# microsoft/crescent-credentials

Measured on AMD Instinct MI355X. Metric: Groth16 proofs/sec (rs256-sd-shaped circuit, BN254), G1 MSM scalar-adds/sec reported alongside, higher is better.
Workload: dtype u32 limbs (BN254 Fq/Fr, 254-bit modular integers)

## Files before the change

### crescent-credentials_amd/csrc/csr_host.hpp

```cpp
#pragma once
#include <string.h>

#include <algorithm>
#include <unordered_map>
#include <vector>

#include "curve.hpp"
#include "errors.hpp"
#include "host_parallel.hpp"

namespace cg {

static constexpr uint32_t SELL_PIECE = 8;
static constexpr uint32_t SELL_FINAL = 0x80000000u;
static constexpr uint32_t SELL_PAD = 0xffffffffu;

struct HostSellLevel {
    uint32_t n_pieces = 0, n_partials = 0;
    std::vector<uint32_t> slice_ptr;
    RawArray<uint32_t> dst, col, cidx;
    size_t n_slots = 0;
};
struct HostCsr {
    uint64_t rows = 0, nnz = 0;
    std::vector<uint32_t> rp;
    RawArray<uint32_t> idx;
    std::vector<Fr> dict_mont;
    std::vector<uint32_t> long_rows;
    std::vector<HostSellLevel> levels;
    uint32_t sell_scratch = 0;
};

inline std::vector<uint64_t> range_bounds(uint64_t n, uint64_t min_chunk) {
    uint64_t parts = std::min<uint64_t>(host_threads(), (n + min_chunk - 1) / (min_chunk ? min_chunk : 1));
    if (parts < 1) parts = 1;
    std::vector<uint64_t> b(parts + 1);
    for (uint64_t k = 0; k <= parts; ++k) b[k] = n * k / parts;
    return b;
}
template <class Fn>
inline void for_ranges(const std::vector<uint64_t>& bounds, Fn fn) {
    const uint64_t parts = bounds.size() - 1;
    parallel_ranges(parts, 1, [&](uint64_t a, uint64_t b) { for (uint64_t k = a; k < b; ++k) fn(k, bounds[k], bounds[k + 1]); });
}

#ifdef CSR_HOST_TIMING
#include <chrono>
#include <stdio.h>
#define CSR_LAP(name) do { auto _n = std::chrono::steady_clock::now(); fprintf(stderr, "    %-28s %.1f ms\n", name, std::chrono::duration<double, std::milli>(_n - _lap).count()); _lap = _n; } while (0)
#define CSR_LAP_START auto _lap = std::chrono::steady_clock::now()
#else
#define CSR_LAP(name) do {} while (0)
#define CSR_LAP_START do {} while (0)
#endif
namespace csr_detail {
struct Key {
    uint64_t w[4];
    bool operator==(const Key& o) const { return !memcmp(w, o.w, 32); }
};
struct KeyHash {
    size_t operator()(const Key& k) const { return (size_t)(k.w[0] * 0x9e3779b97f4a7c15ull ^ k.w[1] ^ (k.w[2] << 1) ^ (k.w[3] << 7)); }
};
}

inline void csr_build_sell_host(HostCsr& out, const uint32_t* col_h, bool reorder);

inline void csr_prepare_host(const cg_csr& m, uint64_t rows, uint64_t num_variables, bool sliced, bool reorder, HostCsr& out) {
    using namespace csr_detail;
    out.rows = rows;
    out.nnz = m.nnz;
    const uint64_t nnz = m.nnz;
    if (nnz >= (1ull << 32)) throw HipError(CG_ERR_INVALID_ARGUMENT, "matrix with >= 2^32 non-zeros");
    if (m.row_ptr[0] != 0 || m.row_ptr[rows] != nnz) throw HipError(CG_ERR_INVALID_ARGUMENT, "row_ptr does not span [0, nnz]");
    CSR_LAP_START;
    out.rp.resize(rows + 1);
    parallel_ranges(rows + 1, 1u << 16, [&](uint64_t lo, uint64_t hi) {
        for (uint64_t i = lo; i < hi; ++i) {
            if (i && m.row_ptr[i] < m.row_ptr[i - 1]) throw HipError(CG_ERR_INVALID_ARGUMENT, "row_ptr not monotone");
            out.rp[i] = (uint32_t)m.row_ptr[i];
        }
    });
    CSR_LAP("row_ptr");
    out.idx.alloc(nnz);
    uint32_t* idx = out.idx.p;
    const std::vector<uint64_t> tb = range_bounds(nnz, 1u << 16);
// ... 11 lines not shown
            Key key;
            memcpy(key.w, m.coeff + 32 * t, 32);
            if (key.w[0] == 1 && !(key.w[1] | key.w[2] | key.w[3])) { idx[t] = 0; continue; }
            if (have_last && key == last) { idx[t] = last_id; continue; }
            auto it = map.find(key);
            if (it == map.end()) {
                it = map.emplace(key, (uint32_t)keys.size()).first;
                keys.push_back(key);
            }
            last = key; last_id = it->second | 0x80000000u; have_last = true;
            idx[t] = last_id;
        }
    });
    CSR_LAP("local dictionaries");
    std::vector<Fr> dict_h;
    {
        Fr o = Fr::zero(); o.l[0] = 1;
        dict_h.push_back(o);
    }
    constexpr uint32_t MERGE_PARTS = 16;
    std::vector<std::vector<uint32_t>> remap(parts);
    for (uint64_t k = 0; k < parts; ++k) remap[k].resize(local_keys[k].size());
    std::vector<std::vector<Key>> class_keys(MERGE_PARTS);
    std::vector<std::exception_ptr> class_err(MERGE_PARTS);
    parallel_ranges(MERGE_PARTS, 1, [&](uint64_t lo, uint64_t hi) {
        for (uint64_t cls = lo; cls < hi; ++cls) {
            std::unordered_map<Key, uint32_t, KeyHash> mine;
            std::vector<Key>& ck = class_keys[cls];
            for (uint64_t k = 0; k < parts; ++k)
                for (size_t j = 0; j < local_keys[k].size(); ++j) {
                    const Key& key = local_keys[k][j];
                    if ((KeyHash()(key) >> 7) % MERGE_PARTS != cls) continue;
                    auto it = mine.find(key);
                    if (it == mine.end()) {
                        bool lt = false;
                        for (int q = 3; q >= 0; --q) {
                            const uint64_t nq = (uint64_t)FrP::N[2 * q] | ((uint64_t)FrP::N[2 * q + 1] << 32);
                            if (key.w[q] != nq) { lt = key.w[q] < nq; break; }
                        }
                        if (!lt) throw HipError(CG_ERR_INVALID_ARGUMENT, "non-canonical matrix coefficient");
                        it = mine.emplace(key, (uint32_t)ck.size()).first;
                        ck.push_back(key);
                    }
                    remap[k][j] = it->second | ((uint32_t)cls << 27);
                }
        }
    });
    uint32_t class_off[MERGE_PARTS + 1];
    class_off[0] = 1;
    for (uint32_t cls = 0; cls < MERGE_PARTS; ++cls) {
        if (class_keys[cls].size() >= (1u << 27)) throw HipError(CG_ERR_INVALID_ARGUMENT, "too many distinct matrix coefficients");
        class_off[cls + 1] = class_off[cls] + (uint32_t)class_keys[cls].size();
    }
    dict_h.resize(class_off[MERGE_PARTS]);
    parallel_ranges(MERGE_PARTS, 1, [&](uint64_t lo, uint64_t hi) {
        for (uint64_t cls = lo; cls < hi; ++cls)
            for (size_t j = 0; j < class_keys[cls].size(); ++j) memcpy(dict_h[class_off[cls] + j].l, class_keys[cls][j].w, 32);
    });
    for (uint64_t k = 0; k < parts; ++k)
        for (uint32_t& v : remap[k]) v = class_off[v >> 27] + (v & ((1u << 27) - 1));
    CSR_LAP("merge");
    for_ranges(tb, [&](uint64_t k, uint64_t lo, uint64_t hi) {
        const uint32_t* rm = remap[k].data();
        for (uint64_t t = lo; t < hi; ++t)
            if (idx[t] & 0x80000000u) idx[t] = rm[idx[t] & 0x7fffffffu];
    });
    parallel_ranges(dict_h.size(), 1u << 12, [&](uint64_t lo, uint64_t hi) { for (uint64_t i = lo; i < hi; ++i) dict_h[i] = to_mont(dict_h[i]); });
    out.dict_mont.swap(dict_h);
    CSR_LAP("remap + to_mont");
    out.long_rows.clear();
    for (uint64_t i = 0; i < rows; ++i)
        if (out.rp[i + 1] - out.rp[i] > 4096u) out.long_rows.push_back((uint32_t)i);
    out.levels.clear();
    out.sell_scratch = 0;
    CSR_LAP("long rows");
    if (sliced) csr_build_sell_host(out, m.col, reorder);
    CSR_LAP("sliced layout");
}

inline void csr_build_sell_host(HostCsr& out, const uint32_t* col_h, bool reorder) {
    struct Item { uint32_t row, first, len; };
    struct Piece { uint32_t first, len, dst; };
    const uint64_t rows = out.rows, nnz = out.nnz;
    const std::vector<uint32_t>& rp = out.rp;
    CSR_LAP_START;
    RawArray<uint32_t> cur_col, cur_idx;
    cur_col.alloc(nnz);
    cur_idx.alloc(nnz);
    parallel_ranges(nnz, 1u << 18, [&](uint64_t lo, uint64_t hi) {
        memcpy(cur_col.p + lo, col_h + lo, (hi - lo) * 4);
        memcpy(cur_idx.p + lo, out.idx.p + lo, (hi - lo) * 4);
    });
    if (reorder)
        parallel_ranges(rows, 1u << 14, [&](uint64_t lo, uint64_t hi) {
            for (uint64_t i = lo; i < hi; ++i) {
                uint32_t w = rp[i];
                for (uint32_t t = rp[i]; t < rp[i + 1]; ++t)
                    if (cur_idx.p[t] != 0) {
                        std::swap(cur_idx.p[t], cur_idx.p[w]);
                        std::swap(cur_col.p[t], cur_col.p[w]);
                        ++w;
                    }
            }
        });
    CSR_LAP("  copy + reorder");
    RawArray<Item> items;
    size_t n_items = 0;
    {
        const std::vector<uint64_t> rb = range_bounds(rows, 1u << 14);
        std::vector<uint64_t> cnt(rb.size(), 0);
        for_ranges(rb, [&](uint64_t k, uint64_t lo, uint64_t hi) {
            uint64_t c = 0;
            for (uint64_t i = lo; i < hi; ++i) c += rp[i + 1] > rp[i];
            cnt[k + 1] = c;
        });
        for (size_t k = 1; k < cnt.size(); ++k) cnt[k] += cnt[k - 1];
        n_items = cnt.back();
        items.alloc(n_items);
        for_ranges(rb, [&](uint64_t k, uint64_t lo, uint64_t hi) {
            uint64_t at = cnt[k];
            for (uint64_t i = lo; i < hi; ++i)
// ... 30 lines not shown
        next_items.alloc(c_next[nr]);
        RawArray<uint32_t> next_col;
        next_col.alloc(partials);
        for_ranges(ib, [&](uint64_t k, uint64_t lo, uint64_t hi) {
            uint64_t p = c_pieces[k], n = c_next[k], q = c_part[k];
            for (uint64_t i = lo; i < hi; ++i) {
                const Item& it = items.p[i];
                const uint32_t np = (it.len + SELL_PIECE - 1) / SELL_PIECE;
                if (np == 1) {
                    pieces.p[p++] = {it.first, it.len, it.row | SELL_FINAL};
                    continue;
                }
                next_items.p[n++] = {it.row, (uint32_t)q, np};
                for (uint32_t j = 0; j < np; ++j) {
                    const uint32_t b = it.first + j * SELL_PIECE;
                    const uint32_t l = it.len - j * SELL_PIECE < SELL_PIECE ? it.len - j * SELL_PIECE : SELL_PIECE;
                    pieces.p[p++] = {b, l, (uint32_t)q};
                    next_col.p[q] = (uint32_t)q;
                    ++q;
                }
            }
        });
        CSR_LAP("  pieces");
        constexpr uint32_t NK = (SELL_PIECE + 1) * (SELL_PIECE + 1);
        auto key_of = [&](const Piece& p) {
            uint32_t k = 0;
            if (reorder)
                for (uint32_t t = 0; t < p.len; ++t) k += cidx[p.first + t] != 0;
            return (SELL_PIECE - k) * (SELL_PIECE + 1) + (SELL_PIECE - p.len);
        };
        const std::vector<uint64_t> pb = range_bounds(n_pieces, 1u << 13);
        const size_t npr = pb.size() - 1;
        RawArray<uint8_t> keys;
        keys.alloc(n_pieces);
        std::vector<uint64_t> hist((npr + 1) * NK, 0);
        for_ranges(pb, [&](uint64_t k, uint64_t lo, uint64_t hi) {
            uint64_t* h = &hist[k * NK];
            for (uint64_t i = lo; i < hi; ++i) { keys.p[i] = (uint8_t)key_of(pieces.p[i]); h[keys.p[i]]++; }
        });
        {
            uint64_t run = 0;
            for (uint32_t key = 0; key < NK; ++key)
                for (size_t k = 0; k < npr; ++k) { const uint64_t c = hist[k * NK + key]; hist[k * NK + key] = run; run += c; }
        }
        for_ranges(pb, [&](uint64_t k, uint64_t lo, uint64_t hi) {
            uint64_t* h = &hist[k * NK];
            for (uint64_t i = lo; i < hi; ++i) sorted.p[h[keys.p[i]]++] = pieces.p[i];
        });
        CSR_LAP("  sort");
        const uint32_t np = (uint32_t)n_pieces, ns = (np + 63) / 64;
        L.slice_ptr.assign(ns + 1, 0);
        L.dst.alloc(np ? np : 1);
        if (!np) L.dst.p[0] = 0;
        parallel_ranges(ns, 1u << 10, [&](uint64_t lo, uint64_t hi) {
            for (uint64_t s = lo; s < hi; ++s) {
                uint32_t longest = 0;
                for (uint32_t p = (uint32_t)s * 64; p < np && p < ((uint32_t)s + 1) * 64; ++p) longest = std::max(longest, sorted.p[p].len);
                L.slice_ptr[s + 1] = 64 * longest;
            }
        });
        for (uint32_t s = 0; s < ns; ++s) L.slice_ptr[s + 1] += L.slice_ptr[s];
// ... 38 lines not shown
```

### crescent-credentials_amd/csrc/field29.hpp

```cpp
#pragma once
#include "field.hpp"

namespace cg {

static constexpr uint32_t M29 = (1u << 29) - 1u;

struct Fq29P {
    static constexpr uint32_t N[9] = {0x187cfd47u, 0x010460b6u, 0x1c72a34fu, 0x02d522d0u, 0x1585d978u,
                                      0x02db40c0u, 0x00a6e141u, 0x0e5c2634u, 0x0030644eu};
    static constexpr uint32_t NINV = 0x04866389u;
    static constexpr uint32_t ONE[9] = {0x157ccc21u, 0x141c2758u, 0x185230d3u, 0x014c0419u, 0x0aa36fb9u,
                                        0x1d4240ceu, 0x11d54c07u, 0x052ac7a8u, 0x000dc836u};
    static constexpr uint32_t R2[9] = {0x059bac10u, 0x0d1503a3u, 0x018016b8u, 0x10ab0ca8u, 0x02632639u,
                                       0x02c0169fu, 0x169bfd53u, 0x11869d4cu, 0x002a11a6u};
    static constexpr uint32_t C256[9] = {0x13349ca1u, 0x1a5d84a8u, 0x0a3e5cacu, 0x100249e0u, 0x12b951e8u,
                                         0x0e92d304u, 0x14cb95b3u, 0x041b9d3du, 0x00058003u};
    typedef FqP P256;
};
struct Fr29P {
    static constexpr uint32_t N[9] = {0x10000001u, 0x1f0fac9fu, 0x0e5c2450u, 0x07d090f3u, 0x1585d283u,
                                      0x02db40c0u, 0x00a6e141u, 0x0e5c2634u, 0x0030644eu};
    static constexpr uint32_t NINV = 0x0fffffffu;
    static constexpr uint32_t ONE[9] = {0x0fffff57u, 0x1ea70ab4u, 0x052c068bu, 0x17504f49u, 0x0aa8075bu,
                                        0x1d4240ceu, 0x11d54c07u, 0x052ac7a8u, 0x000dc836u};
// ... 233 lines not shown
    pack29(t, r.l);
    return r;
}

using Fq29 = F29<Fq29P>;
using Fr29 = F29<Fr29P>;

CG_HD Fr29 weak_reduce(const Fr29& v) {
    constexpr uint32_t MU = 88753990u;
    const uint32_t q = (uint32_t)(((uint64_t)v.l[8] * MU) >> 48);
    const int32_t nq = -(int32_t)q;
    Fr29 r;
    int64_t c = 0;
#pragma unroll
    for (int i = 0; i < 9; ++i) {
        c += (int64_t)v.l[i];
        c += (int64_t)nq * (int64_t)(int32_t)Fr29P::N[i];
        if (i < 8) { r.l[i] = (uint32_t)c & M29; c >>= 29; }
        else r.l[i] = (uint32_t)c;
    }
    return r;
}

CG_HD void bfly(Fr29& u, Fr29& v, const Fr29& w) {
    Fr29 t = mul(v, w);
    v = sub<3, 1>(u, t);
    u = add(u, t);
}

template <class P>
struct S29 {
    int32_t l[9];
    CG_HD static S29 from_unsigned(const F29<P>& a) {
        S29 r;
#pragma unroll
        for (int i = 0; i < 9; ++i) r.l[i] = (int32_t)a.l[i];
        return r;
    }
    CG_HD static S29 one() { return from_unsigned(F29<P>::one()); }
};
struct NoFuse { CG_HD void operator()(int, int64_t&) const {} };
template <class P>
struct FuseMul1 {
    const S29<P>& x; int32_t s;
    CG_HD void operator()(int j, int64_t& c) const { c += (int64_t)x.l[j] * (int64_t)s; }
};
// ... 235 lines not shown
```

### crescent-credentials_amd/csrc/ntt.hip

```cpp

#include "ntt.hpp"

#include <algorithm>

namespace cg {

Fr fr_from_u64(uint64_t v) {
    Fr a = Fr::zero();
    a.l[0] = (uint32_t)v;
    a.l[1] = (uint32_t)(v >> 32);
    return to_mont(a);
}
Fr fr_pow_u64(const Fr& a, uint64_t e) {
    Fr r = Fr::one();
    for (int b = 63; b >= 0; --b) {
        r = sqr(r);
        if ((e >> b) & 1ull) r = mul(r, a);
    }
    return r;
}
Fr fr_root_of_unity(int logn) {
    uint32_t e[8];
    uint32_t nm1[8];
    for (int i = 0; i < 8; ++i) nm1[i] = FrP::N[i];
// ... 83 lines not shown
            uint64_t pos = cur[m.col[t]]++;
            out.row[pos] = (uint32_t)i;
            memcpy(&out.coeff[pos * 32], m.coeff + 32 * t, 32);
        }
    out.view.row_ptr = out.ptr.data();
    out.view.col = out.row.data();
    out.view.coeff = out.coeff.data();
    out.view.nnz = m.nnz;
}


void DevCsr::upload(const cg_csr& m, uint64_t rows_, uint64_t num_variables, hipStream_t st, bool sliced) {
    static const bool plain = CG_TUNE_ENV("SELL_PLAIN") != nullptr;
    HostCsr h;
    csr_prepare_host(m, rows_, num_variables, sliced, !plain, h);
    rows = rows_;
    nnz = m.nnz;
    row_ptr.alloc(rows + 1);
    n_long_rows = h.long_rows.size();
    long_rows.alloc(h.long_rows.size() ? h.long_rows.size() : 1);
    col.alloc(nnz ? nnz : 1);
    coef_idx.alloc(nnz ? nnz : 1);
    dict.alloc(h.dict_mont.size());
    auto h2d = [&](void* dst, const void* src, size_t bytes) { if (bytes) CG_HIP(hipMemcpyAsync(dst, src, bytes, hipMemcpyHostToDevice, st)); };
    h2d(long_rows.p, h.long_rows.data(), h.long_rows.size() * 4);
    h2d(row_ptr.p, h.rp.data(), (rows + 1) * 4);
    h2d(col.p, m.col, nnz * 4);
    h2d(coef_idx.p, h.idx.p, nnz * 4);
    h2d(dict.p, h.dict_mont.data(), h.dict_mont.size() * sizeof(Fr));
    n_sell = (int)h.levels.size();
    sell_scratch = h.sell_scratch;
    for (int k = 0; k < n_sell; ++k) {
        const HostSellLevel& H = h.levels[k];
        SellLevel& L = sell[k];
        L.n_pieces = H.n_pieces;
        L.n_partials = H.n_partials;
        L.slice_ptr.alloc(H.slice_ptr.size()); L.col.alloc(H.n_slots); L.cidx.alloc(H.n_slots); L.dst.alloc(H.dst.size());
        h2d(L.slice_ptr.p, H.slice_ptr.data(), H.slice_ptr.size() * 4);
        h2d(L.col.p, H.col.p, H.n_slots * 4);
        h2d(L.cidx.p, H.cidx.p, H.n_slots * 4);
        h2d(L.dst.p, H.dst.p, H.dst.size() * 4);
    }
    CG_HIP(hipStreamSynchronize(st));
}

static constexpr uint32_t SPMV_LONG_ROW = 4096;

__global__ void __launch_bounds__(256) k_spmv(const uint32_t* __restrict__ row_ptr, const uint32_t* __restrict__ col,
                                              const uint32_t* __restrict__ cidx, const Fr* __restrict__ dict,
                                              const Fr* __restrict__ w, Fr* __restrict__ out, uint64_t rows) {
    uint64_t i = (uint64_t)blockIdx.x * blockDim.x + threadIdx.x;
    if (i >= rows) return;
// ... 45 lines not shown
```

### crescent-credentials_amd/csrc/ntt.hpp

```cpp
#pragma once
#include "common.hpp"
#include "csr_host.hpp"

namespace cg {

struct NttDomain {
    int logn = 0;
    uint64_t n = 0;
    DevBuf<Fr> tw_fwd;
    DevBuf<Fr> tw_inv;
    DevBuf<Fr> coset_br;
    DevBuf<Fr> icoset_br;
    Fr vanishing_inv;
    void build(int logn, bool with_coset, hipStream_t st);
};

Fr fr_from_u64(uint64_t v);
Fr fr_pow_u64(const Fr& a, uint64_t e);
Fr fr_root_of_unity(int logn);

void fr_pow_table(Fr* out, const Fr& base, const Fr& scale, uint64_t n, bool bitrev, int logn, hipStream_t st);

struct SellLevel {
    uint32_t n_pieces = 0, n_partials = 0;
    DevBuf<uint32_t> slice_ptr;
    DevBuf<uint32_t> col;
    DevBuf<uint32_t> cidx;
    DevBuf<uint32_t> dst;
};

struct DevCsr {
    uint64_t rows = 0, nnz = 0;
    DevBuf<uint32_t> row_ptr;
    DevBuf<uint32_t> long_rows;
    uint64_t n_long_rows = 0;
    DevBuf<uint32_t> col;
    DevBuf<uint32_t> coef_idx;
    DevBuf<Fr> dict;
    SellLevel sell[8];
    int n_sell = 0;
    uint32_t sell_scratch = 0;
    void upload(const cg_csr& m, uint64_t rows, uint64_t num_variables, hipStream_t st, bool sliced = true);
};
struct HostCsc {
    std::vector<uint64_t> ptr;
    std::vector<uint32_t> row;
    std::vector<uint8_t> coeff;
    cg_csr view;
};
void csr_transpose(const cg_csr& m, uint64_t rows, uint64_t cols, HostCsc& out);

void spmv(const DevCsr& m, const Fr* w, Fr* out, hipStream_t st);

}
```

### crescent-credentials_amd/csrc/prover.hip

```cpp
#include <atomic>
#include <condition_variable>
#include <shared_mutex>
#include <memory>
#include <mutex>
#include <chrono>
#include <cstdlib>
#include <exception>
#include <functional>
#include <thread>

#include "msm.hpp"
#include "ntt.hpp"
#include "scalar_form.hpp"
#include "wmap29.hpp"

namespace cg {

const char* csr_view_problem(const cg_csr& m);

std::string& last_error() {
    static thread_local std::string e;
    return e;
}
int fail(int code, const char* fmt, ...) {
// ... 721 lines not shown
                    c->b_same_identities = v1 == v2;
                }
            }
        }
        for (const MatJob& j : mj)
            if (j.err) std::rethrow_exception(j.err);
        for (int k = 0; k < 3; ++k) {
            c->matrix_bytes += mj[k].bytes;
            c->lt.matrices_ms = std::max(c->lt.matrices_ms, mj[k].ms);
        }
        {
            AllocScope booking(&c->matrix_bytes);
            if (!c->external_q) {
                c->wdom.build(c->dom, s0);
                if (c->h_strided) c->wstr.build(c->dom, ilog2_ceil((uint64_t)c->shard_count), c->shard_rank, s0);
                c->dA.build(c->A, s0); c->dB.build(c->B, s0); c->dC.build(c->C, s0);
            }
            CG_HIP(hipStreamSynchronize(s0));
            if (c->external_q) {
                c->A = DevCsr(); c->B = DevCsr(); c->C = DevCsr();
            }
            c->dom.tw_fwd.release(); c->dom.tw_inv.release(); c->dom.coset_br.release(); c->dom.icoset_br.release();
            c->A.dict.release(); c->B.dict.release(); c->C.dict.release();
        }
        c->latency = n_slots == 1;
        if (opt && (opt->flags & CG_FLAG_LATENCY_MODE)) c->latency = true;
        if (opt && (opt->flags & CG_FLAG_THROUGHPUT_MODE)) c->latency = false;
        c->spin_wait = opt && (opt->flags & CG_FLAG_SPIN_WAIT);
        if (const char* e = CG_TUNE_ENV("LATENCY_MODE")) c->latency = e[0] == '1';
        const auto t_slots = std::chrono::steady_clock::now();
        const int n_now = staged ? std::min(n_slots, 4) : n_slots;
        if (staged) c->folded = false;
        SlotRecipe slot_recipe;
        for (int k = 0; k < n_now; ++k) c->slots.push_back(make_slot(c.get(), c->tables, s0, slot_recipe));
        CG_HIP(hipStreamSynchronize(s0));
        const char* hwq_env = getenv("GPU_MAX_HW_QUEUES");
        const int hwq = (opt && opt->hw_queues > 0) ? opt->hw_queues : (hwq_env ? atoi(hwq_env) : 4);
        const size_t n_copy_streams = hwq >= n_slots + 4 ? 4 : (size_t)n_slots + 2;
        for (int k = 0; k < n_slots + 2; ++k) {
            if (c->up_streams.size() < n_copy_streams) {
                hipStream_t us = nullptr;
                CG_HIP(hipStreamCreateWithFlags(&us, hipStreamNonBlocking));
                c->up_streams.push_back(us);
            }
            std::unique_ptr<Upload> u(new Upload());
            u->w.alloc(M);
// ... 809 lines not shown
```

### crescent-credentials_amd/csrc/unit.hip

```cpp
#include <chrono>
#include <memory>
#include <mutex>
#include <thread>

#include "host_parallel.hpp"
#include "msm.hpp"
#include "scalar_form.hpp"
#include "wmap29.hpp"

using namespace cg;

struct cg_msm_ctx {
    int device = 0;
    int group = 1;
    uint64_t n = 0;
    bool mont_scalars = false;
    MsmBases<Fq> b1;
    MsmBases<Fq2> b2;
    MsmEngine<Fq> e1;
    MsmEngine<Fq2> e2;
    DevBuf<Fr> scalars;
    DevBuf<uint32_t> bad;
    PinnedBuf<uint32_t> h_bad;
    hipStream_t st = nullptr;
// ... 237 lines not shown
    if (logD > 28)
        return fail(CG_ERR_POLY_DEGREE_TOO_LARGE, "num_constraints + num_inputs = %llu exceeds 2^28",
                    (unsigned long long)(num_constraints + num_inputs));
    try {
        int dev = device;
        if (dev < 0) CG_HIP(hipGetDevice(&dev));
        CG_HIP(hipSetDevice(dev));
        std::unique_ptr<cg_qap_ctx> c(new cg_qap_ctx());
        c->device = dev;
        c->l = num_inputs; c->m = num_constraints; c->M = num_variables;
        c->logD = logD; c->D = 1ull << logD;
        CG_HIP(hipStreamCreateWithFlags(&c->st, hipStreamNonBlocking));
        for (auto& e : c->ev) CG_HIP(hipEventCreate(&e));
        c->A.upload(abc[0], c->m, c->M, c->st);
        c->B.upload(abc[1], c->m, c->M, c->st);
        c->C.upload(abc[2], c->m, c->M, c->st);
        c->dom.build(logD, true, c->st);
        CG_HIP(hipStreamSynchronize(c->st));
        c->wdom.build(c->dom, c->st);
        c->dA.build(c->A, c->st); c->dB.build(c->B, c->st); c->dC.build(c->C, c->st);
        CG_HIP(hipStreamSynchronize(c->st));
        c->dom.tw_fwd.release(); c->dom.tw_inv.release(); c->dom.coset_br.release(); c->dom.icoset_br.release();
        c->A.dict.release(); c->B.dict.release(); c->C.dict.release();
        c->wm.alloc(c->M, c->D, std::max(c->A.sell_scratch, std::max(c->B.sell_scratch, c->C.sell_scratch)));
        c->w_canon.alloc(c->M);
        c->h_canon.alloc(c->D);
        c->mont_scalars = scalar_form == CG_FORM_MONTGOMERY;
        if (c->mont_scalars) c->form_bad.alloc(1);
        *out = c.release();
        return CG_OK;
    } catch (...) {
        return translate_current_exception();
    }
}

extern "C" uint64_t cg_qap_domain_size(const cg_qap_ctx* ctx) { return ctx ? ctx->D : 0; }

static const char* const BAD_ASSIGNMENT = "full_assignment holds a value >= the scalar field modulus";

static const Fr* qap_assignment(cg_qap_ctx* ctx, const void* full_assignment, int on_device) {
    const Fr* w = (const Fr*)full_assignment;
    if (!on_device) {
        CG_HIP(hipMemcpyAsync(ctx->w_canon.p, full_assignment, ctx->M * 32, hipMemcpyHostToDevice, ctx->st));
        w = ctx->w_canon.p;
    }
    if (ctx->mont_scalars) {
// ... 247 lines not shown
```

### crescent-credentials_amd/csrc/wmap29.hip

```cpp
#include "wmap29.hpp"
#include "satcheck.hpp"

namespace cg {

static constexpr int TS29_SMALL = 10, TS29_BIG = 11;
static int strided_max_stages(int tile_log) { return tile_log == TS29_BIG ? 10 : 6; }
static int ntt_passes(int logn, int tile_log) {
    if (logn <= tile_log) return 1;
    const int smax = strided_max_stages(tile_log);
    return 1 + (logn - tile_log + smax - 1) / smax;
}
static int ntt_tile_log(int logn) {
    static const int forced = [] {
        const char* e = CG_TUNE_ENV("NTT_TILE");
        return (e && (atoi(e) == TS29_SMALL || atoi(e) == TS29_BIG)) ? atoi(e) : 0;
    }();
    if (forced) return (forced == TS29_BIG && logn > TS29_SMALL) ? TS29_BIG : TS29_SMALL;
    return (logn >= 20 && ntt_passes(logn, TS29_BIG) < ntt_passes(logn, TS29_SMALL)) ? TS29_BIG : TS29_SMALL;
}

__device__ __forceinline__ Fr29 load_packed29(const uint32_t* __restrict__ base, uint64_t idx) {
    const uint4* p = reinterpret_cast<const uint4*>(base + idx * 8);
    uint4 a = p[0], b = p[1];
    uint32_t w[8] = {a.x, a.y, a.z, a.w, b.x, b.y, b.z, b.w};
// ... 73 lines not shown
    const Fr s = mul(fr_from_u64(5), fr_pow_u64(fr_root_of_unity(big.logn), (uint64_t)rank));
    DevBuf<Fr> t(big.n);
    fr_pow_table(t.p, s, inv(fr_from_u64(big.n)), big.n, false, big.logn, st);
    fold.alloc(big.n * 8);
    k_to_packed29<<<ceil_div(big.n, 256), 256, 0, st>>>(t.p, fold.p, big.n, 0, 0);
    CG_KERNEL_CHECK();
    CG_HIP(hipStreamSynchronize(st));
}

__global__ void __launch_bounds__(256) k_fold29(const uint32_t* __restrict__ a, const uint32_t* __restrict__ T, uint32_t* __restrict__ out,
                                                uint32_t d, int logd, uint32_t terms) {
    const uint32_t i = blockIdx.x * blockDim.x + threadIdx.x;
    if (i >= d) return;
    Fr29 acc = Fr29::zero();
    for (uint32_t t = 0; t < terms; ++t) {
        const uint64_t e = (uint64_t)i + (uint64_t)t * d;
        acc = add(acc, mul(load_packed29(a, e), load_packed29(T, e)));
        if ((t & 3u) == 3u) acc = normalize(acc);
        if ((t & 63u) == 63u) acc = weak_reduce(acc);
    }
    store_packed29(out, brev(i, logd), weak_reduce(normalize(acc)));
}

void Csr29::build(const DevCsr& m, hipStream_t st) {
    dict.alloc(m.dict.n * 8);
    k_to_packed29<<<ceil_div(m.dict.n, 256), 256, 0, st>>>(m.dict.p, dict.p, m.dict.n, 0, 0);
    CG_KERNEL_CHECK();
}

__device__ __forceinline__ bool fr_lt_modulus(const Fr& x) {
    bool lt = false, decided = false;
#pragma unroll
    for (int k = 7; k >= 0; --k) {
        if (!decided && x.l[k] != FrP::N[k]) { lt = x.l[k] < FrP::N[k]; decided = true; }
    }
    return lt;
}

__global__ void __launch_bounds__(256) k_w_to29(const Fr* __restrict__ w, uint32_t* __restrict__ out, uint64_t n,
                                                uint32_t* __restrict__ bad_input, uint32_t* __restrict__ va, uint64_t m, uint64_t l, int logn) {
    uint64_t i = (uint64_t)blockIdx.x * blockDim.x + threadIdx.x;
    if (i >= n) return;
    Fr x = w[i];
    if (!fr_lt_modulus(x)) *bad_input = 1u;
    const Fr29 v = mul(unpack29<Fr29P>(x.l), Fr29::from_limbs(Fr29P::R2));
    store_packed29(out, i, v);
    if (i < l) store_packed29(va, brev((uint32_t)(m + i), logn), v);
}


__global__ void __launch_bounds__(256) k_sell29(const uint32_t* __restrict__ slice_ptr, const uint32_t* __restrict__ col,
                                                const uint32_t* __restrict__ cidx, const uint32_t* __restrict__ dst,
                                                const uint32_t* __restrict__ dict, const uint32_t* __restrict__ src,
                                                uint32_t* __restrict__ out, uint32_t* __restrict__ scratch, uint32_t n_pieces, int logn) {
    const uint32_t p = blockIdx.x * blockDim.x + threadIdx.x;
    if (p >= n_pieces) return;
    const uint32_t s = p >> 6, lane = p & 63u;
    const uint32_t base = slice_ptr[s], len = (slice_ptr[s + 1] - base) >> 6;
    Fr29 acc = Fr29::zero();
    uint32_t cnt = 0;
#if !defined(CG_SELL_BATCH)
#define CG_SELL_BATCH 0
#endif
#if CG_SELL_BATCH == 0
    for (uint32_t t = 0; t < len; ++t) {
        const uint32_t ci = cidx[base + t * 64 + lane];
        if (ci == SELL_PAD) continue;
        Fr29 v = load_packed29(src, col[base + t * 64 + lane]);
        if (ci != 0) v = mul(v, load_packed29(dict, ci));
        acc = add(acc, v);
        if ((++cnt & 3u) == 0) acc = normalize(acc);
    }
#else
    constexpr uint32_t BS = CG_SELL_BATCH;
    uint32_t ci[SELL_PIECE], cl[SELL_PIECE];
#pragma unroll
    for (uint32_t t = 0; t < SELL_PIECE; ++t) {
        const bool in = t < len;
        ci[t] = in ? cidx[base + t * 64 + lane] : SELL_PAD;
        cl[t] = in ? col[base + t * 64 + lane] : 0u;
    }
#pragma unroll
    for (uint32_t h = 0; h < SELL_PIECE; h += BS) {
        if (h >= len) break;
        uint4 rv[BS][2], rd[BS][2];
#pragma unroll
        for (uint32_t u = 0; u < BS; ++u) {
            const uint32_t t = h + u;
            if (ci[t] == SELL_PAD) continue;
            const uint4* pv = reinterpret_cast<const uint4*>(src + (uint64_t)cl[t] * 8);
            rv[u][0] = pv[0]; rv[u][1] = pv[1];
            if (ci[t] != 0) {
                const uint4* pd = reinterpret_cast<const uint4*>(dict + (uint64_t)ci[t] * 8);
                rd[u][0] = pd[0]; rd[u][1] = pd[1];
            }
        }
#pragma unroll
        for (uint32_t u = 0; u < BS; ++u) {
            const uint32_t t = h + u;
            if (ci[t] == SELL_PAD) continue;
            const uint32_t wv[8] = {rv[u][0].x, rv[u][0].y, rv[u][0].z, rv[u][0].w, rv[u][1].x, rv[u][1].y, rv[u][1].z, rv[u][1].w};
            Fr29 v = unpack29<Fr29P>(wv);
            if (ci[t] != 0) {
                const uint32_t wd[8] = {rd[u][0].x, rd[u][0].y, rd[u][0].z, rd[u][0].w, rd[u][1].x, rd[u][1].y, rd[u][1].z, rd[u][1].w};
                v = mul(v, unpack29<Fr29P>(wd));
            }
            acc = add(acc, v);
            if ((++cnt & 3u) == 0) acc = normalize(acc);
        }
    }
#endif
    const uint32_t d = dst[p];
    const Fr29 r = weak_reduce(normalize(acc));
    if (d & SELL_FINAL) store_packed29(out, brev(d & ~SELL_FINAL, logn), r);
    else store_packed29(scratch, d, r);
}

struct Pass29 {
    int logn, ts, S, cbits, gbit_lo, q0;
};
__device__ __forceinline__ uint32_t l2g29(uint32_t e, uint32_t tile, const Pass29& pp) {
    const int extra_bits = pp.ts - pp.S - pp.cbits;
    uint32_t colv = e & ((1u << pp.cbits) - 1u);
    uint32_t g = (e >> pp.cbits) & ((1u << pp.S) - 1u);
    uint32_t extra = e >> (pp.cbits + pp.S);
    uint32_t T = (tile << extra_bits) | extra;
    const int lo_bits = pp.gbit_lo - pp.cbits;
    uint32_t Tlo = T & ((1u << lo_bits) - 1u);
    uint32_t Thi = T >> lo_bits;
    return colv | (Tlo << pp.cbits) | (g << pp.gbit_lo) | (Thi << (pp.gbit_lo + pp.S));
}
__device__ __forceinline__ uint32_t lds_off(uint32_t e) { return e * 9u + (e >> 5); }
__device__ __forceinline__ Fr29 lds_get(const uint32_t* s, uint32_t e) {
    Fr29 r;
    const uint32_t o = lds_off(e);
#pragma unroll
// ... 217 lines not shown
}

static void wm29_products(const Wm29Domain& dom, const DevCsr& A, const DevCsr& B, const DevCsr& C, const Csr29& dA, const Csr29& dB,
                          const Csr29& dC, Wm29Buffers& buf, const Fr* w_canon, uint64_t M, uint64_t m, uint64_t l, hipStream_t st, int nvec,
                          int half) {
    const uint64_t D = dom.n;
    const int logn = dom.logn;
    buf.h_bad_input.p[0] = 0;
    uint32_t* v[3] = {buf.va.p, buf.vb.p, buf.vc.p};
    fill_zero(v[0], D * 32, st);
    k_w_to29<<<ceil_div(M, 256), 256, 0, st>>>(w_canon, buf.w29.p, M, buf.h_bad_input.dev(), buf.va.p, m, l, logn);
    CG_KERNEL_CHECK();
    const DevCsr* mats[3] = {&A, &B, &C};
    const Csr29* dicts[3] = {&dA, &dB, &dC};
    for (int k = 0; k < nvec; ++k) {
        if (half && k != half - 1) continue;
        if (k) fill_zero(v[k], D * 32, st);
        const uint32_t* src = buf.w29.p;
        for (int lv = 0; lv < mats[k]->n_sell; ++lv) {
            const SellLevel& L = mats[k]->sell[lv];
            uint32_t* scratch = (lv & 1) ? buf.sp_b.p : buf.sp_a.p;
            if (L.n_partials > buf.sp_cap) throw HipError(CG_ERR_INVALID_ARGUMENT, "sparse-product scratch smaller than the matrix needs");
            if (L.n_pieces) {
                k_sell29<<<ceil_div(L.n_pieces, 256), 256, 0, st>>>(L.slice_ptr.p, L.col.p, L.cidx.p, L.dst.p, dicts[k]->dict.p, src, v[k],
                                                                    scratch, L.n_pieces, logn);
                CG_KERNEL_CHECK();
            }
            src = scratch;
        }
    }
}
static void wm29_queue_check(const Wm29Domain& dom, Wm29Buffers& buf, uint64_t m, hipStream_t st) {
    k_sat_init29<<<1, 64, 0, st>>>(buf.sat.rec.p);
    k_sat_check29<<<ceil_div(dom.n, 256), 256, 0, st>>>(buf.va.p, buf.vb.p, buf.vc.p, dom.n, m, dom.logn, buf.sat.rec.p);
    CG_KERNEL_CHECK();
    CG_HIP(hipMemcpyAsync(buf.sat.h_rec.p, buf.sat.rec.p, 2 * sizeof(unsigned long long), hipMemcpyDeviceToHost, st));
}

void wm29_check(const Wm29Domain& dom, const DevCsr& A, const DevCsr& B, const DevCsr& C, const Csr29& dA, const Csr29& dB, const Csr29& dC,
                Wm29Buffers& buf, const Fr* w_canon, uint64_t M, uint64_t m, uint64_t l, hipStream_t st) {
    wm29_products(dom, A, B, C, dA, dB, dC, buf, w_canon, M, m, l, st, 3, 0);
    wm29_queue_check(dom, buf, m, st);
    k_sat_row29<<<1, 64, 0, st>>>(buf.va.p, buf.vb.p, buf.vc.p, buf.sat.rec.p, m, dom.logn, buf.sat.row.p);
    CG_KERNEL_CHECK();
    CG_HIP(hipMemcpyAsync(buf.sat.h_row.p, buf.sat.row.p, 24 * sizeof(uint32_t), hipMemcpyDeviceToHost, st));
}

void wm29_run(const Wm29Domain& dom, const DevCsr& A, const DevCsr& B, const DevCsr& C, const Csr29& dA, const Csr29& dB,
// ... 106 lines not shown
```

### crescent-credentials_amd/csrc/wmap29.hpp

```cpp
#pragma once
#include "field29.hpp"
#include "ntt.hpp"

namespace cg {

struct Wm29Domain {
    int logn = 0;
    uint64_t n = 0;
    DevBuf<uint32_t> tw_fwd;
    DevBuf<uint32_t> tw_inv;
    DevBuf<uint32_t> coset;
    DevBuf<uint32_t> icoset;
    uint32_t vinv[8];
    uint32_t vinv_plain[8];
    void build(const NttDomain& d, hipStream_t st);
};

struct Wm29Strided {
    int logs = 0;
    uint64_t d = 0;
    Wm29Domain sub;
    DevBuf<uint32_t> fold;
    void build(const NttDomain& big, int logs, int rank, hipStream_t st);
};

struct Csr29 {
    DevBuf<uint32_t> dict;
    void build(const DevCsr& m, hipStream_t st);
};

struct SatCheck29 {
    DevBuf<unsigned long long> rec;
    PinnedBuf<unsigned long long> h_rec;
    DevBuf<uint32_t> row;
    PinnedBuf<uint32_t> h_row;
    void alloc() { rec.alloc(2); h_rec.alloc(2); row.alloc(24); h_row.alloc(24); }
};

struct Wm29Buffers {
    DevBuf<uint32_t> w29;
    DevBuf<uint32_t> va, vb, vc, vt;
    DevBuf<uint32_t> sp_a, sp_b;
    uint32_t sp_cap = 0;
    PinnedBuf<uint32_t> h_bad_input;
    SatCheck29 sat;
    void alloc(uint64_t M, uint64_t D, uint32_t sparse_scratch) {
        w29.alloc(M * 8); va.alloc(D * 8); vb.alloc(D * 8); vc.alloc(D * 8); vt.alloc(D * 8);
        sp_cap = sparse_scratch;
        sp_a.alloc((size_t)(sparse_scratch ? sparse_scratch : 1) * 8); sp_b.alloc((size_t)(sparse_scratch ? sparse_scratch : 1) * 8);
        h_bad_input.alloc(1);
// ... 26 lines not shown
```

Measured before the change: 180.2.

## Use signed small-integer coefficient path with lazy column reduction in sparse matvec

```diff
diff --git a/crescent-credentials_amd/csrc/csr_host.hpp b/crescent-credentials_amd/csrc/csr_host.hpp
--- a/crescent-credentials_amd/csrc/csr_host.hpp
+++ b/crescent-credentials_amd/csrc/csr_host.hpp
@@ -26,6 +26,9 @@
     std::vector<uint32_t> rp;
     RawArray<uint32_t> idx;
     std::vector<Fr> dict_mont;
+    std::vector<int32_t> small;
+    uint32_t n_small1 = 1;
+    uint64_t census[3] = {0, 0, 0};
     std::vector<uint32_t> long_rows;
     std::vector<HostSellLevel> levels;
     uint32_t sell_scratch = 0;
@@ -61,6 +64,20 @@
 struct KeyHash {
     size_t operator()(const Key& k) const { return (size_t)(k.w[0] * 0x9e3779b97f4a7c15ull ^ k.w[1] ^ (k.w[2] << 1) ^ (k.w[3] << 7)); }
 };
+}
+
+static constexpr uint32_t SELL_SMALL_BITS = 29;
+inline int32_t csr_small_coeff(const uint64_t c[4]) {
+    if (!(c[1] | c[2] | c[3])) return c[0] < (1ull << SELL_SMALL_BITS) ? (int32_t)c[0] : 0;
+    uint64_t d[4], borrow = 0;
+    for (int q = 0; q < 4; ++q) {
+        const uint64_t nq = (uint64_t)FrP::N[2 * q] | ((uint64_t)FrP::N[2 * q + 1] << 32);
+        const uint64_t t = nq - c[q];
+        d[q] = t - borrow;
+        borrow = (nq < c[q]) | (t < borrow);
+    }
+    if (borrow || (d[1] | d[2] | d[3]) || d[0] >= (1ull << SELL_SMALL_BITS)) return 0;
+    return -(int32_t)d[0];
 }
 
 inline void csr_build_sell_host(HostCsr& out, const uint32_t* col_h, bool reorder);
@@ -118,6 +135,7 @@
     std::vector<std::vector<uint32_t>> remap(parts);
     for (uint64_t k = 0; k < parts; ++k) remap[k].resize(local_keys[k].size());
     std::vector<std::vector<Key>> class_keys(MERGE_PARTS);
+    std::vector<std::vector<int32_t>> class_small(MERGE_PARTS);
     std::vector<std::exception_ptr> class_err(MERGE_PARTS);
     parallel_ranges(MERGE_PARTS, 1, [&](uint64_t lo, uint64_t hi) {
         for (uint64_t cls = lo; cls < hi; ++cls) {
@@ -137,30 +155,58 @@
                         if (!lt) throw HipError(CG_ERR_INVALID_ARGUMENT, "non-canonical matrix coefficient");
                         it = mine.emplace(key, (uint32_t)ck.size()).first;
                         ck.push_back(key);
+                        class_small[cls].push_back(csr_small_coeff(key.w));
                     }
                     remap[k][j] = it->second | ((uint32_t)cls << 27);
                 }
         }
     });
-    uint32_t class_off[MERGE_PARTS + 1];
-    class_off[0] = 1;
+    uint32_t small_off[MERGE_PARTS + 1], gen_off[MERGE_PARTS + 1];
+    small_off[0] = 1;
     for (uint32_t cls = 0; cls < MERGE_PARTS; ++cls) {
         if (class_keys[cls].size() >= (1u << 27)) throw HipError(CG_ERR_INVALID_ARGUMENT, "too many distinct matrix coefficients");
-        class_off[cls + 1] = class_off[cls] + (uint32_t)class_keys[cls].size();
+        uint32_t ns = 0;
+        for (int32_t v : class_small[cls]) ns += v != 0;
+        small_off[cls + 1] = small_off[cls] + ns;
     }
-    dict_h.resize(class_off[MERGE_PARTS]);
+    const uint32_t n_small1 = small_off[MERGE_PARTS];
+    gen_off[0] = n_small1;
+    for (uint32_t cls = 0; cls < MERGE_PARTS; ++cls) gen_off[cls + 1] = gen_off[cls] + (uint32_t)class_keys[cls].size() - (small_off[cls + 1] - small_off[cls]);
+    dict_h.resize(gen_off[MERGE_PARTS]);
+    out.n_small1 = n_small1;
+    out.small.assign(n_small1, 0);
+    out.small[0] = 1;
+    std::vector<std::vector<uint32_t>> class_final(MERGE_PARTS);
     parallel_ranges(MERGE_PARTS, 1, [&](uint64_t lo, uint64_t hi) {
-        for (uint64_t cls = lo; cls < hi; ++cls)
-            for (size_t j = 0; j < class_keys[cls].size(); ++j) memcpy(dict_h[class_off[cls] + j].l, class_keys[cls][j].w, 32);
+        for (uint64_t cls = lo; cls < hi; ++cls) {
+            uint32_t s_at = small_off[cls], g_at = gen_off[cls];
+            class_final[cls].resize(class_keys[cls].size());
+            for (size_t j = 0; j < class_keys[cls].size(); ++j) {
+                const int32_t sv = class_small[cls][j];
+                const uint32_t at = sv ? s_at++ : g_at++;
+                if (sv) out.small[at] = sv;
+                class_final[cls][j] = at;
+                memcpy(dict_h[at].l, class_keys[cls][j].w, 32);
+            }
+        }
     });
     for (uint64_t k = 0; k < parts; ++k)
-        for (uint32_t& v : remap[k]) v = class_off[v >> 27] + (v & ((1u << 27) - 1));
+        for (uint32_t& v : remap[k]) v = class_final[v >> 27][v & ((1u << 27) - 1)];
     CSR_LAP("merge");
+    std::vector<uint64_t> cens(parts * 3, 0);
     for_ranges(tb, [&](uint64_t k, uint64_t lo, uint64_t hi) {
         const uint32_t* rm = remap[k].data();
-        for (uint64_t t = lo; t < hi; ++t)
+        uint64_t n_one = 0, n_small = 0;
+        for (uint64_t t = lo; t < hi; ++t) {
             if (idx[t] & 0x80000000u) idx[t] = rm[idx[t] & 0x7fffffffu];
-    });
+            n_one += idx[t] == 0;
+            n_small += idx[t] < n_small1;
+        }
+        cens[3 * k] = n_one; cens[3 * k + 1] = n_small - n_one; cens[3 * k + 2] = (hi - lo) - n_small;
+    });
+    out.census[0] = out.census[1] = out.census[2] = 0;
+    for (uint64_t k = 0; k < parts; ++k)
+        for (int q = 0; q < 3; ++q) out.census[q] += cens[3 * k + q];
     parallel_ranges(dict_h.size(), 1u << 12, [&](uint64_t lo, uint64_t hi) { for (uint64_t i = lo; i < hi; ++i) dict_h[i] = to_mont(dict_h[i]); });
     out.dict_mont.swap(dict_h);
     CSR_LAP("remap + to_mont");
@@ -187,12 +233,21 @@
         memcpy(cur_col.p + lo, col_h + lo, (hi - lo) * 4);
         memcpy(cur_idx.p + lo, out.idx.p + lo, (hi - lo) * 4);
     });
+    const uint32_t n_small1 = out.n_small1;
     if (reorder)
         parallel_ranges(rows, 1u << 14, [&](uint64_t lo, uint64_t hi) {
             for (uint64_t i = lo; i < hi; ++i) {
                 uint32_t w = rp[i];
                 for (uint32_t t = rp[i]; t < rp[i + 1]; ++t)
                     if (cur_idx.p[t] != 0) {
+                        std::swap(cur_idx.p[t], cur_idx.p[w]);
+                        std::swap(cur_col.p[t], cur_col.p[w]);
+                        ++w;
+                    }
+                const uint32_t products_end = w;
+                w = rp[i];
+                for (uint32_t t = rp[i]; t < products_end; ++t)
+                    if (cur_idx.p[t] >= n_small1) {
                         std::swap(cur_idx.p[t], cur_idx.p[w]);
                         std::swap(cur_col.p[t], cur_col.p[w]);
                         ++w;
@@ -269,21 +324,21 @@
             }
         });
         CSR_LAP("  pieces");
-        constexpr uint32_t NK = (SELL_PIECE + 1) * (SELL_PIECE + 1);
+        constexpr uint32_t NK = (SELL_PIECE + 1) * (SELL_PIECE + 1) * (SELL_PIECE + 1);
         auto key_of = [&](const Piece& p) {
-            uint32_t k = 0;
+            uint32_t k = 0, g = 0;
             if (reorder)
-                for (uint32_t t = 0; t < p.len; ++t) k += cidx[p.first + t] != 0;
-            return (SELL_PIECE - k) * (SELL_PIECE + 1) + (SELL_PIECE - p.len);
+                for (uint32_t t = 0; t < p.len; ++t) { k += cidx[p.first + t] != 0; g += cidx[p.first + t] >= n_small1; }
+            return ((SELL_PIECE - k) * (SELL_PIECE + 1) + (SELL_PIECE - p.len)) * (SELL_PIECE + 1) + (SELL_PIECE - g);
         };
         const std::vector<uint64_t> pb = range_bounds(n_pieces, 1u << 13);
         const size_t npr = pb.size() - 1;
-        RawArray<uint8_t> keys;
+        RawArray<uint16_t> keys;
         keys.alloc(n_pieces);
         std::vector<uint64_t> hist((npr + 1) * NK, 0);
         for_ranges(pb, [&](uint64_t k, uint64_t lo, uint64_t hi) {
             uint64_t* h = &hist[k * NK];
-            for (uint64_t i = lo; i < hi; ++i) { keys.p[i] = (uint8_t)key_of(pieces.p[i]); h[keys.p[i]]++; }
+            for (uint64_t i = lo; i < hi; ++i) { keys.p[i] = (uint16_t)key_of(pieces.p[i]); h[keys.p[i]]++; }
         });
         {
             uint64_t run = 0;
diff --git a/crescent-credentials_amd/csrc/field29.hpp b/crescent-credentials_amd/csrc/field29.hpp
--- a/crescent-credentials_amd/csrc/field29.hpp
+++ b/crescent-credentials_amd/csrc/field29.hpp
@@ -279,6 +279,36 @@
     return r;
 }
 
+CG_HD uint64_t mulhi64(uint64_t a, uint64_t b) {
+    const uint64_t a0 = (uint32_t)a, a1 = a >> 32, b0 = (uint32_t)b, b1 = b >> 32;
+    const uint64_t p01 = a0 * b1, p10 = a1 * b0;
+    const uint64_t mid = ((a0 * b0) >> 32) + (uint32_t)p01 + (uint32_t)p10;
+    return a1 * b1 + (p01 >> 32) + (p10 >> 32) + (mid >> 32);
+}
+static constexpr int COLS29_LOGK = 36;
+static constexpr uint64_t COLS29_KN_TOP = 0x30644e72e131a02ull;
+static constexpr uint64_t COLS29_MU = 0xa948e8c4c474094full;
+CG_HD Fr29 reduce_columns(const int64_t (&col)[9]) {
+    const uint64_t T = (uint64_t)(col[8] + (col[7] >> 29) - 10) + COLS29_KN_TOP;
+    const int64_t q = (int64_t)(mulhi64(T << 5, COLS29_MU) >> 26) - ((int64_t)1 << COLS29_LOGK);
+    const int32_t nq0 = -(int32_t)((uint32_t)q & M29), nq1 = -(int32_t)(q >> 29);
+    Fr29 r;
+    int64_t c = 0;
+#pragma unroll
+    for (int i = 0; i < 9; ++i) {
+        c += col[i];
+        c += (int64_t)nq0 * (int64_t)(int32_t)Fr29P::N[i];
+        if (i) c += (int64_t)nq1 * (int64_t)(int32_t)Fr29P::N[i - 1];
+        if (i < 8) { r.l[i] = (uint32_t)c & M29; c >>= 29; }
+        else r.l[i] = (uint32_t)c + ((uint32_t)(nq1 * (int32_t)Fr29P::N[8]) << 29);
+    }
+    return r;
+}
+CG_HD void mad_columns(int64_t (&col)[9], const Fr29& v, int32_t s) {
+#pragma unroll
+    for (int i = 0; i < 9; ++i) col[i] += (int64_t)(int32_t)v.l[i] * (int64_t)s;
+}
+
 CG_HD void bfly(Fr29& u, Fr29& v, const Fr29& w) {
     Fr29 t = mul(v, w);
     v = sub<3, 1>(u, t);
diff --git a/crescent-credentials_amd/csrc/ntt.hip b/crescent-credentials_amd/csrc/ntt.hip
--- a/crescent-credentials_amd/csrc/ntt.hip
+++ b/crescent-credentials_amd/csrc/ntt.hip
@@ -129,12 +129,15 @@
     col.alloc(nnz ? nnz : 1);
     coef_idx.alloc(nnz ? nnz : 1);
     dict.alloc(h.dict_mont.size());
+    small.alloc(h.small.size());
+    n_small1 = h.n_small1;
     auto h2d = [&](void* dst, const void* src, size_t bytes) { if (bytes) CG_HIP(hipMemcpyAsync(dst, src, bytes, hipMemcpyHostToDevice, st)); };
     h2d(long_rows.p, h.long_rows.data(), h.long_rows.size() * 4);
     h2d(row_ptr.p, h.rp.data(), (rows + 1) * 4);
     h2d(col.p, m.col, nnz * 4);
     h2d(coef_idx.p, h.idx.p, nnz * 4);
     h2d(dict.p, h.dict_mont.data(), h.dict_mont.size() * sizeof(Fr));
+    h2d(small.p, h.small.data(), h.small.size() * 4);
     n_sell = (int)h.levels.size();
     sell_scratch = h.sell_scratch;
     for (int k = 0; k < n_sell; ++k) {
diff --git a/crescent-credentials_amd/csrc/ntt.hpp b/crescent-credentials_amd/csrc/ntt.hpp
--- a/crescent-credentials_amd/csrc/ntt.hpp
+++ b/crescent-credentials_amd/csrc/ntt.hpp
@@ -37,6 +37,8 @@
     DevBuf<uint32_t> col;
     DevBuf<uint32_t> coef_idx;
     DevBuf<Fr> dict;
+    DevBuf<int32_t> small;
+    uint32_t n_small1 = 1;
     SellLevel sell[8];
     int n_sell = 0;
     uint32_t sell_scratch = 0;
diff --git a/crescent-credentials_amd/csrc/prover.hip b/crescent-credentials_amd/csrc/prover.hip
--- a/crescent-credentials_amd/csrc/prover.hip
+++ b/crescent-credentials_amd/csrc/prover.hip
@@ -767,6 +767,7 @@
             }
             c->dom.tw_fwd.release(); c->dom.tw_inv.release(); c->dom.coset_br.release(); c->dom.icoset_br.release();
             c->A.dict.release(); c->B.dict.release(); c->C.dict.release();
+            c->A.small.release(); c->B.small.release(); c->C.small.release();
         }
         c->latency = n_slots == 1;
         if (opt && (opt->flags & CG_FLAG_LATENCY_MODE)) c->latency = true;
diff --git a/crescent-credentials_amd/csrc/unit.hip b/crescent-credentials_amd/csrc/unit.hip
--- a/crescent-credentials_amd/csrc/unit.hip
+++ b/crescent-credentials_amd/csrc/unit.hip
@@ -283,6 +283,7 @@
         CG_HIP(hipStreamSynchronize(c->st));
         c->dom.tw_fwd.release(); c->dom.tw_inv.release(); c->dom.coset_br.release(); c->dom.icoset_br.release();
         c->A.dict.release(); c->B.dict.release(); c->C.dict.release();
+        c->A.small.release(); c->B.small.release(); c->C.small.release();
         c->wm.alloc(c->M, c->D, std::max(c->A.sell_scratch, std::max(c->B.sell_scratch, c->C.sell_scratch)));
         c->w_canon.alloc(c->M);
         c->h_canon.alloc(c->D);
diff --git a/crescent-credentials_amd/csrc/wmap29.hip b/crescent-credentials_amd/csrc/wmap29.hip
--- a/crescent-credentials_amd/csrc/wmap29.hip
+++ b/crescent-credentials_amd/csrc/wmap29.hip
@@ -119,10 +119,21 @@
     store_packed29(out, brev(i, logd), weak_reduce(normalize(acc)));
 }
 
+__global__ void __launch_bounds__(256) k_small_to_dict(const int32_t* __restrict__ small, uint32_t* __restrict__ dict, uint32_t n_small1) {
+    const uint32_t i = blockIdx.x * blockDim.x + threadIdx.x + 1u;
+    if (i < n_small1) dict[(uint64_t)i * 8] = (uint32_t)small[i];
+}
+
 void Csr29::build(const DevCsr& m, hipStream_t st) {
     dict.alloc(m.dict.n * 8);
     k_to_packed29<<<ceil_div(m.dict.n, 256), 256, 0, st>>>(m.dict.p, dict.p, m.dict.n, 0, 0);
     CG_KERNEL_CHECK();
+    n_small1 = m.n_small1;
+    if (n_small1 > 1) {
+        if (m.small.n < n_small1 || m.dict.n < n_small1) throw HipError(CG_ERR_INVALID_ARGUMENT, "small-coefficient table shorter than its range");
+        k_small_to_dict<<<ceil_div(n_small1 - 1, 256), 256, 0, st>>>(m.small.p, dict.p, n_small1);
+        CG_KERNEL_CHECK();
+    }
 }
 
 __device__ __forceinline__ bool fr_lt_modulus(const Fr& x) {
@@ -148,67 +159,38 @@
 
 __global__ void __launch_bounds__(256) k_sell29(const uint32_t* __restrict__ slice_ptr, const uint32_t* __restrict__ col,
                                                 const uint32_t* __restrict__ cidx, const uint32_t* __restrict__ dst,
-                                                const uint32_t* __restrict__ dict, const uint32_t* __restrict__ src,
+                                                const uint32_t* __restrict__ dict, uint32_t n_small1, const uint32_t* __restrict__ src,
                                                 uint32_t* __restrict__ out, uint32_t* __restrict__ scratch, uint32_t n_pieces, int logn) {
     const uint32_t p = blockIdx.x * blockDim.x + threadIdx.x;
     if (p >= n_pieces) return;
     const uint32_t s = p >> 6, lane = p & 63u;
     const uint32_t base = slice_ptr[s], len = (slice_ptr[s + 1] - base) >> 6;
     Fr29 acc = Fr29::zero();
+    int64_t wide[9] = {0, 0, 0, 0, 0, 0, 0, 0, 0};
+    bool any_small = false;
     uint32_t cnt = 0;
-#if !defined(CG_SELL_BATCH)
-#define CG_SELL_BATCH 0
-#endif
-#if CG_SELL_BATCH == 0
     for (uint32_t t = 0; t < len; ++t) {
         const uint32_t ci = cidx[base + t * 64 + lane];
         if (ci == SELL_PAD) continue;
         Fr29 v = load_packed29(src, col[base + t * 64 + lane]);
+        if (ci != 0 && ci < n_small1) {
+            mad_columns(wide, v, (int32_t)dict[(uint64_t)ci * 8]);
+            any_small = true;
+            continue;
+        }
         if (ci != 0) v = mul(v, load_packed29(dict, ci));
         acc = add(acc, v);
         if ((++cnt & 3u) == 0) acc = normalize(acc);
     }
-#else
-    constexpr uint32_t BS = CG_SELL_BATCH;
-    uint32_t ci[SELL_PIECE], cl[SELL_PIECE];
+    const uint32_t d = dst[p];
+    Fr29 r;
+    if (any_small) {
 #pragma unroll
-    for (uint32_t t = 0; t < SELL_PIECE; ++t) {
-        const bool in = t < len;
-        ci[t] = in ? cidx[base + t * 64 + lane] : SELL_PAD;
-        cl[t] = in ? col[base + t * 64 + lane] : 0u;
-    }
-#pragma unroll
-    for (uint32_t h = 0; h < SELL_PIECE; h += BS) {
-        if (h >= len) break;
-        uint4 rv[BS][2], rd[BS][2];
-#pragma unroll
-        for (uint32_t u = 0; u < BS; ++u) {
-            const uint32_t t = h + u;
-            if (ci[t] == SELL_PAD) continue;
-            const uint4* pv = reinterpret_cast<const uint4*>(src + (uint64_t)cl[t] * 8);
-            rv[u][0] = pv[0]; rv[u][1] = pv[1];
-            if (ci[t] != 0) {
-                const uint4* pd = reinterpret_cast<const uint4*>(dict + (uint64_t)ci[t] * 8);
-                rd[u][0] = pd[0]; rd[u][1] = pd[1];
-            }
-        }
-#pragma unroll
-        for (uint32_t u = 0; u < BS; ++u) {
-            const uint32_t t = h + u;
-            if (ci[t] == SELL_PAD) continue;
-            const uint32_t wv[8] = {rv[u][0].x, rv[u][0].y, rv[u][0].z, rv[u][0].w, rv[u][1].x, rv[u][1].y, rv[u][1].z, rv[u][1].w};
-            Fr29 v = unpack29<Fr29P>(wv);
-            if (ci[t] != 0) {
-                const uint32_t wd[8] = {rd[u][0].x, rd[u][0].y, rd[u][0].z, rd[u][0].w, rd[u][1].x, rd[u][1].y, rd[u][1].z, rd[u][1].w};
-                v = mul(v, unpack29<Fr29P>(wd));
-            }
-            acc = add(acc, v);
-            if ((++cnt & 3u) == 0) acc = normalize(acc);
-        }
-    }
-#endif
-    const uint32_t d = dst[p];
-    const Fr29 r = weak_reduce(normalize(acc));
+        for (int i = 0; i < 9; ++i) wide[i] += (int64_t)acc.l[i];
+        r = reduce_columns(wide);
+    } else {
+        r = weak_reduce(normalize(acc));
+    }
     if (d & SELL_FINAL) store_packed29(out, brev(d & ~SELL_FINAL, logn), r);
     else store_packed29(scratch, d, r);
 }
@@ -472,8 +454,8 @@
             uint32_t* scratch = (lv & 1) ? buf.sp_b.p : buf.sp_a.p;
             if (L.n_partials > buf.sp_cap) throw HipError(CG_ERR_INVALID_ARGUMENT, "sparse-product scratch smaller than the matrix needs");
             if (L.n_pieces) {
-                k_sell29<<<ceil_div(L.n_pieces, 256), 256, 0, st>>>(L.slice_ptr.p, L.col.p, L.cidx.p, L.dst.p, dicts[k]->dict.p, src, v[k],
-                                                                    scratch, L.n_pieces, logn);
+                k_sell29<<<ceil_div(L.n_pieces, 256), 256, 0, st>>>(L.slice_ptr.p, L.col.p, L.cidx.p, L.dst.p, dicts[k]->dict.p, dicts[k]->n_small1,
+                                                                    src, v[k], scratch, L.n_pieces, logn);
                 CG_KERNEL_CHECK();
             }
             src = scratch;
diff --git a/crescent-credentials_amd/csrc/wmap29.hpp b/crescent-credentials_amd/csrc/wmap29.hpp
--- a/crescent-credentials_amd/csrc/wmap29.hpp
+++ b/crescent-credentials_amd/csrc/wmap29.hpp
@@ -26,6 +26,7 @@
 
 struct Csr29 {
     DevBuf<uint32_t> dict;
+    uint32_t n_small1 = 1;
     void build(const DevCsr& m, hipStream_t st);
 };
 
```

Result: slower. 175.7 (-2.5%).
